# FlinkML/flink-parameter-server

Measured on NVIDIA H100. Metric: matrix-factorization updates/sec (whole box, max over ranks), higher is better.
Workload: dtype fp32

## Files before the change

### flink-parameter-server_b200/models/mf/device.py

```python
from __future__ import annotations

import math
import os
from typing import Iterable, Optional, Sequence, Tuple

import torch
import torch.distributed as dist

from ...errors import FactorIsNotANumberException
from ...ops import native
from ...utils.metrics import GLOBAL as METRICS
from ...runtime.device_stream import DevicePrefetcher
from ...store.replica_cache import ReplicaCache
from ...store.sharded_table import ShardedTable

ERR_SIGMOID = 0
ERR_PLAIN = 1

DEFAULT_DEVICE_PULL_LIMIT = 0

L2_TABLE_BYTES = 48 << 20
WINDOW_BUDGET = 256 << 20
WINDOW_BYTES_PER_ROW = 8 + 12
WINDOW_MAX_STRIDE = 128
# ... 88 lines not shown
                 flush_require: str = "any", replica_own_inplace: Optional[bool] = None,
                 output_ring=None, loss: str = "pointwise", regularization: float = 0.0,
                 step_window: Optional[int] = None, optimizer: str = "sgd",
                 negative_sampling: str = "uniform", margin: Optional[float] = None):
        self._pending = []
        self.step_window = 0
        check_negative_sampling(negative_sampling, negative_sample_rate)
        self.negative_sampling = negative_sampling
        if loss not in ("pointwise", "bpr", "warp"):
            raise ValueError(f"loss must be 'pointwise', 'bpr' or 'warp', got {loss!r}")
        self.loss, self.reg = loss, float(regularization)
        if loss == "pointwise" and self.reg != 0.0:
            raise ValueError("regularization is only supported with loss='bpr' or loss='warp'")
        self.margin = check_warp(loss, margin, optimizer=optimizer, negative_sampling=negative_sampling)
        if loss != "pointwise":
            if output_ring is not None:
                raise ValueError(f"the per-update output ring is not supported with loss={loss!r}")
            if kernel == "tma":
                raise ValueError(f"kernel='tma' is not supported with loss={loss!r}")
            if item_blocking:
                raise ValueError(f"item_blocking is not supported with loss={loss!r}")
            item_blocking = False
        self.device = torch.cuda.current_device() if device is None else int(device)
        self.cuda_device = torch.device("cuda", self.device)
        self.group = group
        ready = dist.is_available() and dist.is_initialized()
        self.world = dist.get_world_size(group) if ready else 1
        self.rank = dist.get_rank(group) if ready else 0
        if item_cache is None:
            item_cache = self.world > 1 and os.environ.get("FPS_ITEM_CACHE", "1") != "0"
        check_optimizer(optimizer, item_cache=bool(item_cache), output_ring=output_ring, kernel=kernel)
        self.optimizer = optimizer
        self.num_users, self.num_items, self.k = int(num_users), int(num_items), int(num_factors)
        self.lr = float(learning_rate)
        self.neg = int(negative_sample_rate)
        self.pull_limit = int(pull_limit)
        self.err_mode = int(err_mode)
        self.seed = int(seed)
        self.step_no = 0
        self.kernel = kernel
        self.credits = (torch.tensor([self.pull_limit, 0], dtype=torch.int32, device=self.cuda_device)
                        if self.pull_limit >= 32 and os.environ.get("FPS_STATIC_LIMITER", "0") != "1"
                        and loss == "pointwise" and optimizer == "sgd" else None)
        self.output_ring = output_ring
        with torch.cuda.device(self.device):
            self._items = ShardedTable(num_items, num_factors, partition="hash", group=group,
                                      device=self.device, init="uniform",
                                      init_range=(range_min, range_max), seed=seed * 2 + 1,
                                      track_touched=track_touched)
            n_local = -(-self.num_users // self.world)
            self._users = torch.empty((n_local, self._items.stride), dtype=torch.float32,
                                     device=self.cuda_device)
            native.init_rows(self._users, self.k, self.rank, self.world, native.PART_HASH, n_local,
                             seed * 2 + 2, range_min, range_max)
            self._stats = torch.zeros(STATS_SIZE[loss], dtype=torch.float32, device=self.cuda_device)
            self._user_acc = self._item_acc = None
            if optimizer == "adagrad":
                self._user_acc = torch.zeros(n_local, dtype=torch.float32, device=self.cuda_device)
                self._item_acc = self._items.row_accumulators()
            self._nan_flag = torch.zeros(1, dtype=torch.int32, device=self.cuda_device)
            self.user_memory = int(user_memory) if self.neg > 0 else 0
            if self.user_memory > 0:
                self.seen = torch.full((n_local, self.user_memory), -1, dtype=torch.int32,
                                       device=self.cuda_device)
                self.seen_pos = torch.zeros(n_local, dtype=torch.int32, device=self.cuda_device)
            self._registry = (native.seen_registry(self.num_items, self.cuda_device)
                              if negative_sampling == "seen" else None)
        self.item_cache = bool(item_cache)
        self.sync_every = max(1, int(sync_every))
        self.sync_interval_ms = sync_interval_ms
        self.flush_count, self.flush_require = flush_count, flush_require
        self._own_inplace = replica_own_inplace
        self.replica = (ReplicaCache(self._items, self.sync_every, sync_interval_ms,
                                     require=flush_require, flush_count=flush_count,
                                     own_inplace=replica_own_inplace)
                        if self.item_cache else None)
        row_bytes = self._items.stride * 4
        if item_blocking is None:
            item_blocking = ((self.world == 1 or self.item_cache) and self.num_items * row_bytes > (48 << 20)
                             and (self.neg == 0 or self.user_memory > 0 or negative_sampling == "seen")
                             and os.environ.get("FPS_ITEM_BLOCKING", "1") != "0")
        self.item_blocking = bool(item_blocking)
        block_bytes = int(os.environ.get("FPS_BLOCK_BYTES", block_bytes))
        self.l2_hints = self.item_blocking and os.environ.get("FPS_L2_HINTS", "0") == "1"
        per_bucket = max(1, int(block_bytes) // row_bytes)
        self.block_shift = max(0, per_bucket.bit_length() - 1)
        table_rows = self._items.rows_per_shard * self.world if self.item_cache else self.num_items
        self._table_rows = table_rows
        while -(-table_rows >> self.block_shift) > native.BUCKET_MAX:
            self.block_shift += 1
        self.block_buckets = max(1, -(-table_rows >> self.block_shift))
        if self.item_blocking:
            with torch.cuda.device(self.device):
                self._bucket_scratch = torch.zeros(2 * native.BUCKET_MAX, dtype=torch.int32,
                                                   device=self.cuda_device)
        self.step_window = step_window_size(step_window, world=self.world, item_cache=self.item_cache,
                                            loss=self.loss, table_rows=self.num_items, stride=self._items.stride,
                                            env=os.environ.get("FPS_STEP_WINDOW"), optimizer=optimizer)
        self._win = None
        self._win_phase_ns = None
        self._graph_capture = False
        self._per_launch = False
        self._items.barrier()

    @property
    def stats(self) -> torch.Tensor:
        self._drain()
        return self._stats

    @property
    def users(self) -> torch.Tensor:
        self._drain()
        return self._users

    @property
    def items(self) -> ShardedTable:
        self._drain()
        return self._items

    @property
    def nan_flag(self) -> torch.Tensor:
        self._drain()
        return self._nan_flag

    @property
    def accumulators(self) -> Optional[Tuple[torch.Tensor, torch.Tensor]]:
        self._drain()
        if self._item_acc is None:
            return None
        return self._user_acc, self._item_acc.local

    def _windowable(self, users, items, ratings) -> bool:
        if self.step_window < 2 or self._graph_capture or self._per_launch:
            return False
        packed = items is None
        return step_windowable(
            neg=self.neg, output_ring=self.output_ring, pull_limit=self.pull_limit, credits=self.credits,
            kernel=self.kernel, kernel_env=os.environ.get("FPS_MF_KERNEL", "reg"),
            reg_variant_env=os.environ.get("FPS_MF_REG_VARIANT"), l2_hints=self.l2_hints, packed=packed,
            dtypes=(users.dtype,) if packed else (users.dtype, items.dtype, ratings.dtype),
            n_records=users.numel(), table_rows=self.num_items, on_gpu=users.is_cuda,
            capturing=torch.cuda.is_current_stream_capturing())

    def _stage(self, users, items, ratings) -> None:
        if self._win is None:
            rows, w = self.num_items, self.step_window
            slot_bytes = -(-rows * 12 // 256) * 256
            with torch.cuda.device(self.device):
                dev = self.cuda_device
                self._win = {
                    "slot_bytes": slot_bytes,
                    "stage": torch.empty(w * slot_bytes, dtype=torch.uint8, device=dev),
                    "slots": torch.full((w, rows), -1, dtype=torch.int64, device=dev),
                    "user_bits": torch.zeros(-(-self._users.shape[0] // 32), dtype=torch.int32, device=dev),
                    "ctl": torch.zeros(2 * native.WINDOW_MAX, dtype=torch.int32, device=dev),
                    "slot_stats": torch.zeros((w, 2), dtype=torch.float32, device=dev),
                }
        j = len(self._pending)
        n = users.numel()
        sb = self._win["slot_bytes"]
        slot = self._win["stage"][j * sb:(j + 1) * sb]
        if items is None:
            slot[:8 * n].view(torch.int64).copy_(users.reshape(-1), non_blocking=True)
        else:
            ids = slot[:12 * n].view(torch.int32)
            ids[:n].copy_(users.reshape(-1), non_blocking=True)
            ids[n:2 * n].copy_(items.reshape(-1), non_blocking=True)
            ids[2 * n:].view(torch.float32).copy_(ratings.reshape(-1), non_blocking=True)
        self._pending.append((n, 1 if items is None else 0))
        self.step_no += 1
        METRICS.inc("mf_ratings", n)

    def _drain(self) -> int:
        n = len(self._pending)
        if n == 0:
            return 0
        counts, fmts = zip(*self._pending)
        self._pending = []
        w = self._win
        native.mf_window_drain(w["stage"], w["slot_bytes"], counts, fmts, self._users, self._items.local, self.lr,
                               self.err_mode, w["slots"], w["user_bits"], w["ctl"], self._stats, w["slot_stats"],
                               self._nan_flag, phase_ns=self._win_phase_ns)
        return n

    def flush(self) -> None:
        self._drain()
        if self.replica is not None:
            self.replica.flush()

    def step(self, users: torch.Tensor, items: Optional[torch.Tensor] = None,
             ratings: Optional[torch.Tensor] = None, negatives: Optional[torch.Tensor] = None) -> None:
        if self.loss == "pointwise" and negatives is None and self._windowable(users, items, ratings):
            self._stage(users, items, ratings)
            if len(self._pending) >= self.step_window:
                self._drain()
            return
        self._drain()
        check_negative_sampling(self.negative_sampling, self.neg, negatives)
        if self.loss != "pointwise":
            self._step_pairwise(users, items, ratings, negatives)
            return
        if negatives is not None:
            raise ValueError("negatives= needs loss='bpr' or loss='warp'")
        neg = self.neg
        if self.user_memory > 0 or self._registry is not None:
            users, items, ratings = self._sample_negatives(users, items, ratings)
            neg = 0
        n_records = users.numel()
        fed = False
        ring = self.output_ring
        out_args = ring.kernel_args() if ring is not None else None
        revisits = self.item_cache or n_records * (1 + neg) > self._table_rows
        if self.item_blocking and self.block_buckets > 1 and revisits:
            hashed = self.item_cache and self._items.mode == native.PART_HASH
            fed = hashed
            users, items, ratings = native.bucket_by_item(
                users, items, ratings, self.block_shift, self.block_buckets, self._bucket_scratch,
                num_shards=self.world if hashed else 1, rows_per_shard=self._items.rows_per_shard,
                pending=self.replica.pending if hashed else None)
        if self.item_cache:
            self.replica.after_step(n_records * (1 + neg), fed=fed)
            native.mf_sgd_fused(users, items, ratings, self._users, self.world, self.replica.table_c,
                                self.lr, err_mode=self.err_mode, neg_rate=neg,
                                num_items=self.num_items, seed=self.seed, step=self.step_no,
                                stats=self._stats, nan_flag=self._nan_flag,
                                max_inflight_rows=self.pull_limit, kernel="reg", l2_hints=self.l2_hints,
                                reserve_total=self.replica.reserve_total(), output=out_args,
                                credits=self.credits)
        else:
            native.mf_sgd_fused(users, items, ratings, self._users, self.world, self._items.table_c,
                                self.lr, err_mode=self.err_mode, neg_rate=neg,
                                num_items=self.num_items, seed=self.seed, step=self.step_no,
                                stats=self._stats, nan_flag=self._nan_flag,
                                max_inflight_rows=self.pull_limit, kernel=self.kernel,
                                l2_hints=self.l2_hints, output=out_args, credits=self.credits,
                                item_acc=self._item_acc.table_c if self._item_acc is not None else None,
                                user_acc=self._user_acc)
        if ring is not None:
            ring.after_kernel(users.numel() * (1 + neg))
        self.step_no += 1
        METRICS.inc("mf_ratings", users.numel())

    def _step_pairwise(self, users, items, ratings, negatives) -> None:
        if negatives is not None:
            if self.item_cache:
                raise ValueError("negatives= is not supported in the replica (item_cache) mode")
            n = int(negatives.shape[1]) if negatives.dim() == 2 else 0
        elif self.neg < 1:
            raise ValueError(f"loss={self.loss!r} needs negative_sample_rate >= 1 or explicit negatives=")
        elif self.user_memory > 0 or self._registry is not None:
            per = 1 + self.neg
            ou, oi, orat = self._sample_negatives(users, items, ratings)
            ou, oi = ou.view(-1, per), oi.view(-1, per)
            negatives = torch.where(ou[:, 1:] >= 0, oi[:, 1:], torch.full_like(oi[:, 1:], -1)).contiguous()
            users, items, ratings = ou[:, 0].contiguous(), oi[:, 0].contiguous(), orat.view(-1, per)[:, 0].contiguous()
            n = self.neg
        else:
            n = self.neg
        if self.output_ring is not None:
            raise ValueError(f"the per-update output ring is not supported with loss={self.loss!r}")
        n_pos = users.numel()
        cand, reserve = self._items.table_c, 0
        if self.item_cache:
            self.replica.after_step(n_pos * (n if self.loss == "bpr" else 1), fed=False)
            cand, reserve = self.replica.table_c, self.replica.reserve_total()
        if self.loss == "warp":
            native.mf_warp_fused(users, items, ratings, self._users, cand, self.lr, self.reg, margin=self.margin,
                                 rank_items=self.num_items, negatives=negatives, n_neg=n, num_items=self.num_items,
                                 seed=self.seed, step=self.step_no, anchor_div=self.world, stats=self._stats,
                                 nan_flag=self._nan_flag, max_inflight_rows=self.pull_limit, reserve_total=reserve)
            self.step_no += 1
            METRICS.inc("mf_ratings", n_pos)
            return
        native.mf_bpr_fused(users, items, ratings, self._users, cand, self.lr, self.reg, negatives=negatives,
                            n_neg=n, num_items=self.num_items, seed=self.seed, step=self.step_no,
                            anchor_div=self.world, stats=self._stats, nan_flag=self._nan_flag,
                            max_inflight_rows=self.pull_limit, reserve_total=reserve,
                            anchor_acc=self._user_acc,
                            cand_acc=self._item_acc.table_c if self._item_acc is not None else None)
        self.step_no += 1
        METRICS.inc("mf_ratings", n_pos)

    def _sample_negatives(self, users, items, ratings):
        memory = self.user_memory > 0
        if self._registry is not None:
            return native.neg_sample_seen(users, items, ratings, self.neg, self._registry,
                                          self.seen if memory else None, self.seen_pos if memory else None,
                                          self.world, seed=self.seed, step=self.step_no)
        return native.neg_sample(users, items, ratings, self.neg, self.num_items, self.seen, self.seen_pos,
                                 self.world, seed=self.seed, step=self.step_no)

    def seen_items(self) -> torch.Tensor:
        if self._registry is None:
            raise ValueError("seen_items() needs negative_sampling='seen'")
        order, count, _ = self._registry
        return order[:int(count.item())].to(torch.int64)

    def make_graph_step(self, batch_size: int, packed: bool = True):
        self._drain()
        dev = self.cuda_device
        if packed:
            static = (torch.zeros(batch_size, dtype=torch.int64, device=dev),)
        else:
            static = (torch.zeros(batch_size, dtype=torch.int32, device=dev),
                      torch.zeros(batch_size, dtype=torch.int32, device=dev),
                      torch.zeros(batch_size, dtype=torch.float32, device=dev))
        s = torch.cuda.Stream(device=dev)
        s.wait_stream(torch.cuda.current_stream(dev))
        self._graph_capture = True
        try:
            with torch.cuda.stream(s):
                for _ in range(2):
                    self._stats.zero_(); self.step(*static)
            torch.cuda.current_stream(dev).wait_stream(s)
            graph = torch.cuda.CUDAGraph()
            with torch.cuda.graph(graph, stream=s):
                self._stats.zero_()
                self.step(*static)
        finally:
            self._graph_capture = False

        def replay():
            self._drain()
            graph.replay()
        return static, replay

    def fit_stream(self, host_batches: Iterable[Sequence[torch.Tensor]],
                   loss_every: int = 1):
        self._drain()
        pf = DevicePrefetcher(host_batches, self.cuda_device, depth=2)
        self.prefetcher = pf
        pending = []
        ring = [torch.empty(self._stats.numel(), dtype=torch.float32).pin_memory() for _ in range(4)]
        i = 0
        for batch in pf:
# ... 100 lines not shown
```

### flink-parameter-server_b200/ops/csrc/fps_mf_window.cu

```cuda
#include <cuda_fp16.h>
#include <cooperative_groups.h>
#include "fps_common.cuh"
#include "fps_mf_args.cuh"

namespace cg = cooperative_groups;

#define WIN_MAX 8
#define WIN_THREADS 256
#define WIN_EMPTY 0xFFFFFFFFFFFFFFFFull

struct WinArgs {
  const unsigned char* stage;
  long long slot_bytes;
  long long n[WIN_MAX];
  int fmt[WIN_MAX];
  int n_slots;
  int err_mode;
  float lr;
  int stride;
  float* user_table;
  float* item_table;
  long long rows;
  unsigned long long* slots;
  unsigned int* user_bits;
  long long bm_words;
  unsigned int* ctl;
  float* stats;
  float* slot_stats;
  int* nan_flag;
  unsigned long long* phase_ns;
};

__device__ __forceinline__ bool win_record(const WinArgs& a, int j, long long i, int& user, int& item,
                                           float& rating) {
  const unsigned char* base = a.stage + (long long)j * a.slot_bytes;
  if (a.fmt[j] == 1) {
    const unsigned long long rec = reinterpret_cast<const unsigned long long*>(base)[i];
    user = (int)(rec >> 38);
    item = (int)((rec >> 16) & 0x3FFFFFull);
    rating = __half2float(__ushort_as_half((unsigned short)(rec & 0xFFFFull)));
    return true;
  }
  const long long n = a.n[j];
  user = reinterpret_cast<const int*>(base)[i];
  item = reinterpret_cast<const int*>(base)[n + i];
  rating = reinterpret_cast<const float*>(base)[2 * n + i];
  return user >= 0;
}

__device__ __forceinline__ float win_add(float x, float y) {
  float z;
  asm("add.rn.ftz.f32 %0, %1, %2;" : "=f"(z) : "f"(x), "f"(y));
  return z;
}
__device__ __forceinline__ float4 win_add4(float4 x, float g, float4 y) {
  return make_float4(win_add(x.x, g * y.x), win_add(x.y, g * y.y), win_add(x.z, g * y.z), win_add(x.w, g * y.w));
}

__device__ __forceinline__ unsigned long long win_clock() {
  unsigned long long t;
  asm volatile("mov.u64 %0, %%globaltimer;" : "=l"(t));
  return t;
}
__device__ __forceinline__ void win_phase(const WinArgs& a, int k) {
  const unsigned long long t = win_clock();
  a.phase_ns[k] += t - a.phase_ns[3];
  a.phase_ns[3] = t;
  if (k == 1) a.phase_ns[2] += 1ull;
}

template <int G, int NS>
__device__ __forceinline__ void win_flush_stats(const WinArgs& a, float (&sq)[NS], float (&cnt)[NS], int nr,
                                                int slot0, float* sh) {
  const int lane = threadIdx.x & (G - 1);
  __syncthreads();
  if (threadIdx.x < 2 * WIN_MAX) sh[threadIdx.x] = 0.f;
  __syncthreads();
#pragma unroll
  for (int r = 0; r < WIN_MAX; ++r) {
    if (r < nr) {
      const bool mine = lane == r % G;
      float s = mine ? sq[r / G] : 0.f, c = mine ? cnt[r / G] : 0.f;
#pragma unroll
      for (int o = 16; o > 0; o >>= 1) {
        s += __shfl_xor_sync(0xffffffffu, s, o);
        c += __shfl_xor_sync(0xffffffffu, c, o);
      }
      if ((threadIdx.x & 31) == 0 && c > 0.f) {
        atomicAdd(sh + 2 * r, s);
        atomicAdd(sh + 2 * r + 1, c);
      }
    }
  }
#pragma unroll
  for (int i = 0; i < NS; ++i) sq[i] = cnt[i] = 0.f;
  __syncthreads();
  if (threadIdx.x < 2 * nr && sh[threadIdx.x] != 0.f)
    atomicAdd(a.slot_stats + 2 * slot0 + threadIdx.x, sh[threadIdx.x]);
}

template <int G, int VPL>
__device__ __forceinline__ void win_load(float4 (&x)[VPL], const float* row, int lane, int nvec, bool on) {
#pragma unroll
  for (int k = 0; k < VPL; ++k) {
    const int c = lane + k * G;
    x[k] = (on && c < nvec) ? *reinterpret_cast<const float4*>(row + 4 * c) : make_float4(0.f, 0.f, 0.f, 0.f);
  }
}
template <int G, int VPL>
__device__ __forceinline__ void win_store(float* row, const float4 (&x)[VPL], int lane, int nvec) {
#pragma unroll
  for (int k = 0; k < VPL; ++k) {
    const int c = lane + k * G;
    if (c < nvec) *reinterpret_cast<float4*>(row + 4 * c) = x[k];
  }
}
template <int G, int VPL>
__device__ __forceinline__ float win_dot(const float4 (&u)[VPL], const float4 (&v)[VPL]) {
  float d[VPL];
#pragma unroll
  for (int k = 0; k < VPL; ++k) {
    d[k] = 0.f;
    d[k] += fps_mf_dot4(u[k], v[k]);
  }
#pragma unroll
  for (int h = VPL / 2; h > 0; h >>= 1)
#pragma unroll
    for (int k = 0; k < h; ++k) d[k] += d[k + h];
  return fps_group_sum<G>(d[0]);
}

template <int LPR, int VPL, int P, int MINB>
__global__ void __launch_bounds__(WIN_THREADS, MINB) fps_mf_window_kernel(const __grid_constant__ WinArgs a) {
  static_assert(VPL >= 1 && VPL <= LPR && LPR % VPL == 0, "VPL must divide LPR");
  constexpr int G = LPR / VPL;
  __shared__ float sh[2 * WIN_MAX];
  cg::grid_group grid = cg::this_grid();
  const int lane = threadIdx.x & (G - 1);
  const int gtid = blockIdx.x * blockDim.x + threadIdx.x;
  const int gthreads = gridDim.x * blockDim.x;
  const int group = gtid / G;
  const int n_groups = gthreads / G;
  const int stride = a.stride;
  const int nvec = stride >> 2;
  constexpr int NS = G < WIN_MAX ? WIN_MAX / G : 1;
  constexpr int NE = NS;
  float sq[NS], cnt[NS];
#pragma unroll
  for (int i = 0; i < NS; ++i) sq[i] = cnt[i] = 0.f;
  bool bad = false;
  const bool timer = a.phase_ns != nullptr && blockIdx.x == 0 && threadIdx.x == 0;

  if (blockIdx.x == 0) {
    if (threadIdx.x < 2 * WIN_MAX) a.ctl[threadIdx.x] = 0u;
    if (threadIdx.x < 2 * a.n_slots) a.slot_stats[threadIdx.x] = 0.f;
  }
  if (timer) a.phase_ns[3] = win_clock();
  int start = 0, attempt = 0;
  while (start < a.n_slots) {
    for (long long w = gtid; w < a.bm_words; w += gthreads) a.user_bits[w] = 0u;
    grid.sync();
    int end = start;
    bool clashed = false;
    while (end < a.n_slots) {
      const int j = end;
      unsigned long long* t = a.slots + (long long)(j - start) * a.rows;
      bool clash = false;
      for (long long i = gtid; i < a.n[j]; i += gthreads) {
        int user, item;
        float rating;
        if (!win_record(a, j, i, user, item, rating)) continue;
        const unsigned long long e = ((unsigned long long)__float_as_uint(rating) << 32) | (unsigned int)user;
        clash |= atomicExch(t + item, e) != WIN_EMPTY;
        const unsigned int bit = 1u << (user & 31);
        clash |= (atomicOr(a.user_bits + (user >> 5), bit) & bit) != 0u;
      }
      if (clash) *reinterpret_cast<volatile unsigned int*>(a.ctl + attempt) = 1u;
      grid.sync();
      clashed = *reinterpret_cast<volatile unsigned int*>(a.ctl + attempt) != 0u;
      ++attempt;
      if (clashed) break;
      ++end;
    }
    if (timer) win_phase(a, 0);
    const int nrow = end - start;
    const int written = nrow + (clashed ? 1 : 0);
    if (nrow > 0) {
      unsigned long long nxt[NE];
#pragma unroll
      for (int m = 0; m < NE; ++m) {
        const int r = lane + m * G;
        nxt[m] = (group < a.rows && r < written) ? a.slots[(long long)r * a.rows + group] : WIN_EMPTY;
      }
      for (long long base = 0; base < a.rows; base += n_groups) {
        const long long item = base + group;
        const bool in = item < a.rows;
        float* vp = a.item_table + (in ? item : 0) * (long long)stride;
        float4 v[VPL];
#pragma unroll
        for (int k = 0; k < VPL; ++k) v[k] = make_float4(0.f, 0.f, 0.f, 0.f);
        bool any = false;
        bool loaded = false;
        unsigned long long mine[NE];
#pragma unroll
        for (int m = 0; m < NE; ++m) {
          const int r = lane + m * G;
          mine[m] = nxt[m];
          const long long it2 = item + n_groups;
          nxt[m] = (it2 < a.rows && r < written) ? a.slots[(long long)r * a.rows + it2] : WIN_EMPTY;
          if (mine[m] != WIN_EMPTY) a.slots[(long long)r * a.rows + item] = WIN_EMPTY;
        }
        const int src0 = (threadIdx.x & 31) & ~(G - 1);
#pragma unroll
        for (int c0 = 0; c0 < WIN_MAX; c0 += P) {
          if (c0 < nrow) {
            unsigned long long ent[P];
#pragma unroll
            for (int q = 0; q < P; ++q) {
              const int r = c0 + q;
              ent[q] = __shfl_sync(0xffffffffu, mine[(r / G) % NE], src0 + r % G);
              if (r >= nrow) ent[q] = WIN_EMPTY;
            }
            {
              bool chunk_any = false;
#pragma unroll
              for (int q = 0; q < P; ++q) chunk_any |= ent[q] != WIN_EMPTY;
              if (chunk_any && !loaded) win_load<G, VPL>(v, vp, lane, nvec, true);
              loaded |= chunk_any;
              any |= chunk_any;
              float4 u[P][VPL];
#pragma unroll
              for (int q = 0; q < P; ++q)
                win_load<G, VPL>(u[q], a.user_table + (long long)(unsigned int)ent[q] * stride, lane, nvec,
                                 ent[q] != WIN_EMPTY);
#pragma unroll
              for (int q = 0; q < P; ++q) {
                const int r = c0 + q;
                if (r < nrow) {
                  const float d = win_dot<G, VPL>(u[q], v);
                  const bool ok = ent[q] != WIN_EMPTY;
                  const float rating = __uint_as_float((unsigned int)(ent[q] >> 32));
                  const float resid = rating - d;
                  const float g = fps_mf_grad(a.err_mode, a.lr, rating, d, resid);
                  if (ok) {
                    if (!(fabsf(g) <= 3.0e38f)) bad = true;
                    if (lane == r % G) {
                      sq[r / G] += resid * resid;
                      cnt[r / G] += 1.f;
                    }
                    float4 nu[VPL];
#pragma unroll
                    for (int k = 0; k < VPL; ++k) {
                      nu[k] = win_add4(u[q][k], g, v[k]);
                      v[k] = win_add4(v[k], g, u[q][k]);
                    }
                    win_store<G, VPL>(a.user_table + (long long)(unsigned int)ent[q] * stride, nu, lane, nvec);
                  }
                }
              }
            }
          }
        }
        if (any) win_store<G, VPL>(vp, v, lane, nvec);
      }
      win_flush_stats<G, NS>(a, sq, cnt, nrow, start, sh);
    } else {
      const int j = start;
      unsigned long long* t = a.slots;
      for (long long base = 0; base < a.n[j]; base += n_groups) {
        const long long i = base + group;
        int user = 0, item = 0;
        float rating = 0.f;
        const bool ok = i < a.n[j] && win_record(a, j, i, user, item, rating);
        float* up = a.user_table + (long long)user * stride;
        float* vp = a.item_table + (long long)item * stride;
        float4 u[VPL], v[VPL];
#pragma unroll
        for (int k = 0; k < VPL; ++k) {
          const int c = lane + k * G;
          u[k] = v[k] = make_float4(0.f, 0.f, 0.f, 0.f);
          if (ok && c < nvec) {
            v[k] = fps_ld_row4(vp + 4 * c);
            u[k] = *reinterpret_cast<const float4*>(up + 4 * c);
          }
        }
        const float d = win_dot<G, VPL>(u, v);
        const float resid = rating - d;
        const float g = fps_mf_grad(a.err_mode, a.lr, rating, d, resid);
        if (ok) {
          if (!(fabsf(g) <= 3.0e38f)) bad = true;
          if (lane == 0) {
            sq[0] += resid * resid;
            cnt[0] += 1.f;
            t[item] = WIN_EMPTY;
          }
#pragma unroll
          for (int k = 0; k < VPL; ++k) {
            const int c = lane + k * G;
            if (c < nvec) {
              fps_red_add4(up + 4 * c, make_float4(g * v[k].x, g * v[k].y, g * v[k].z, g * v[k].w));
              fps_red_add4(vp + 4 * c, make_float4(g * u[k].x, g * u[k].y, g * u[k].z, g * u[k].w));
            }
          }
        }
      }
      win_flush_stats<G, NS>(a, sq, cnt, 1, start, sh);
      end = start + 1;
    }
    grid.sync();
    if (timer) win_phase(a, 1);
    start = end;
  }
  if (bad && a.nan_flag != nullptr) *a.nan_flag = 1;
  if (blockIdx.x == 0 && threadIdx.x == 0 && a.stats != nullptr) {
    float s = 0.f, c = 0.f;
    for (int j = 0; j < a.n_slots; ++j) {
      s += a.slot_stats[2 * j];
      c += a.slot_stats[2 * j + 1];
    }
    a.stats[0] += s;
    a.stats[1] += c;
  }
}

template <int LPR, int VPL, int P, int MINB>
static int launch_window(const WinArgs& a, int num_sms, cudaStream_t stream) {
  constexpr int V = VPL < LPR ? VPL : LPR;
  int occ = 0;
  cudaError_t e =
      cudaOccupancyMaxActiveBlocksPerMultiprocessor(&occ, fps_mf_window_kernel<LPR, V, P, MINB>, WIN_THREADS, 0);
  if (e != cudaSuccess) return (int)e;
  if (occ < 1) return -1402;
  const long long grid = (long long)num_sms * occ;
  WinArgs args = a;
  void* params[] = {&args};
  e = cudaLaunchCooperativeKernel((const void*)fps_mf_window_kernel<LPR, V, P, MINB>, dim3((unsigned)grid),
                                  dim3(WIN_THREADS), params, 0, stream);
  if (e != cudaSuccess) return (int)e;
  return (int)cudaGetLastError();
}

static int g_win_variant = 0;
extern "C" void fps_set_mf_window_variant(int v) { g_win_variant = v; }

template <int LPR>
static int dispatch_window(const WinArgs& a, int num_sms, cudaStream_t s) {
  constexpr int MINB_V1 = LPR <= 2 ? 2 : 3;
  switch (g_win_variant) {
    case 1: return launch_window<LPR, 1, 8, 1>(a, num_sms, s);
    case 2: return launch_window<LPR, 1, 4, MINB_V1>(a, num_sms, s);
    default:
      if constexpr (LPR == 16) return launch_window<16, 4, 2, 2>(a, num_sms, s);
      else return launch_window<LPR, 1, 4, MINB_V1>(a, num_sms, s);
  }
}

extern "C" int fps_mf_window_drain(const WinArgs* a, int num_sms, cudaStream_t stream) {
  if (a->n_slots <= 0) return 0;
  if (a->n_slots > WIN_MAX) return -1401;
  const int nvec = a->stride >> 2;
  if (nvec <= 1) return dispatch_window<1>(*a, num_sms, stream);
  if (nvec <= 2) return dispatch_window<2>(*a, num_sms, stream);
  if (nvec <= 4) return dispatch_window<4>(*a, num_sms, stream);
  if (nvec <= 8) return dispatch_window<8>(*a, num_sms, stream);
  if (nvec <= 16) return dispatch_window<16>(*a, num_sms, stream);
  if (nvec <= 32) return dispatch_window<32>(*a, num_sms, stream);
  return -1400;
}
```

### flink-parameter-server_b200/ops/native.py

```python
from __future__ import annotations

import ctypes as C
import math
import os
import threading
from typing import Optional

import torch

from . import build as _build

FPS_MAX_SHARDS = 16
PART_HASH = 0
PART_RANGE = 1
PART_LUT = 2
LUT_OWNER_SHIFT = 40

_lib = None
_lib_lock = threading.Lock()
_launch_count = 0


class ShardTableC(C.Structure):

# ... 161 lines not shown

class _RawCudaBuffer:

    def __init__(self, ptr: int, shape, typestr: str):
        self.__cuda_array_interface__ = {
            "shape": tuple(shape),
            "typestr": typestr,
            "data": (int(ptr), False),
            "version": 3,
            "strides": None,
        }


_TYPESTR = {torch.float32: "<f4", torch.int32: "<i4", torch.int64: "<i8", torch.uint8: "|u1",
            torch.float16: "<f2", torch.int16: "<i2"}


def tensor_from_ptr(ptr: int, shape, dtype: torch.dtype, device: int) -> torch.Tensor:
    if dtype == torch.bfloat16:
        t = torch.as_tensor(_RawCudaBuffer(ptr, shape, "<i2"), device=torch.device("cuda", device))
        return t.view(torch.bfloat16)
    return torch.as_tensor(_RawCudaBuffer(ptr, shape, _TYPESTR[dtype]),
                           device=torch.device("cuda", device))


def init_rows(rows: torch.Tensor, dim: int, shard: int, num_shards: int, mode: int, div: int,
              seed: int, lo: float, hi: float) -> None:
    _req(rows, "rows", torch.float32)
    n_rows, stride = rows.shape
    assert stride % 4 == 0
    _check(lib().fps_init_rows(C.c_void_p(rows.data_ptr()), C.c_longlong(n_rows), int(dim),
                               int(stride), int(shard), int(num_shards), int(mode),
                               C.c_longlong(div), C.c_ulonglong(seed & (2**64 - 1)),
                               C.c_float(lo), C.c_float(hi), _stream()), "init_rows")
    _bump()


MF_ERR_MODES = (0, 1, 2)


def _check_pointwise(users, items, ratings, err_mode) -> None:
    if int(err_mode) not in MF_ERR_MODES:
        raise ValueError(f"err_mode must be one of {MF_ERR_MODES}, got {err_mode!r}")
    if items is None:
        if users.dtype != torch.int64:
            raise TypeError("packed rating records must be an int64 tensor (see pack_ratings)")
        return
    if users.dtype != items.dtype:
        raise TypeError("users and items must share an integer dtype")
    if items.numel() != users.numel() or ratings.numel() != users.numel():
        raise ValueError("users, items and ratings must have the same length")


def mf_sgd_fused(users: torch.Tensor, items: torch.Tensor, ratings: torch.Tensor,
                 user_table, user_div: int, item_tab: ShardTableC, lr: float,
                 err_mode: int = 0, neg_rate: int = 0, num_items: int = 0, seed: int = 0,
                 step: int = 0, stats: Optional[torch.Tensor] = None,
                 nan_flag: Optional[torch.Tensor] = None, max_inflight_rows: int = 0,
                 kernel: Optional[str] = None, push_tab: Optional[ShardTableC] = None,
                 l2_hints: bool = False, reserve_ctas: int = 0, reserve_total: int = 0,
                 progress: Optional[torch.Tensor] = None, output=None,
                 credits: Optional[torch.Tensor] = None, item_acc: Optional[ShardTableC] = None,
                 user_acc=None) -> None:
    _check_pointwise(users, items, ratings, err_mode)
    if int(neg_rate) > 0 and int(num_items) < 2:
        raise ValueError(f"sampled negatives need num_items >= 2, got {num_items}")
    _req(users, "users")
    user_sharded = isinstance(user_table, ShardTableC)
    if not user_sharded:
        _req(user_table, "user_table", torch.float32)
    packed = items is None
    if not packed:
        _req(items, "items"); _req(ratings, "ratings", torch.float32)
    if (user_table.stride if user_sharded else user_table.shape[1]) != item_tab.stride:
        raise ValueError("user table stride must equal item table stride")
    a = MfArgsC()
    a.users = users.data_ptr()
    a.items = None if packed else items.data_ptr()
    a.ratings = None if packed else ratings.data_ptr()
    a.format = 1 if packed else 0
    a.n_pos = users.numel(); a.neg_rate = int(neg_rate); a.num_items = int(max(num_items, 1))
    a.seed = seed & (2**64 - 1); a.step = int(step)
    if user_sharded:
        a.user_table = None; a.user_tab = user_table; a.user_sharded = 1
    else:
        a.user_table = user_table.data_ptr(); a.user_sharded = 0
    a.user_div = int(user_div)
    a.user_shift = log2_or_neg(int(user_div))
    a.lr = float(lr); a.err_mode = int(err_mode)
    a.stats = stats.data_ptr() if stats is not None else None
    a.nan_flag = nan_flag.data_ptr() if nan_flag is not None else None
    a.item_tab = item_tab
    if push_tab is not None:
        a.push_tab = push_tab; a.use_push_tab = 1
    a.l2_hints = 1 if l2_hints else 0
    variant = kernel or os.environ.get("FPS_MF_KERNEL", "reg")
    if packed or push_tab is not None or l2_hints or output is not None or credits is not None:
        variant = "reg"
    a.progress = progress.data_ptr() if progress is not None else None
    if credits is not None:
        _req(credits, "credits", torch.int32)
        a.credits = credits.data_ptr()
    if output is not None:
        o_ids, o_vecs, o_staged, o_cap, o_every = output
        a.out_ids = o_ids.data_ptr(); a.out_vecs = o_vecs.data_ptr(); a.out_staged = o_staged.data_ptr()
        a.out_cap = int(o_cap); a.out_every = int(o_every)
    if item_acc is not None:
        if push_tab is not None or output is not None or credits is not None:
            raise ValueError("row-wise AdaGrad does not support push_tab, output or credits")
        if int(item_acc.stride) != 1:
            raise ValueError("item_acc must be a stride-1 accumulator table")
        a.item_acc = item_acc
        if user_sharded:
            if not isinstance(user_acc, ShardTableC) or int(user_acc.stride) != 1:
                raise ValueError("a sharded user table needs a stride-1 ShardTableC user_acc")
            a.user_acc_tab = user_acc
        else:
            if not torch.is_tensor(user_acc):
                raise ValueError("a worker-local user table needs a float32 user_acc tensor")
            _req(user_acc, "user_acc", torch.float32)
            if user_acc.numel() < user_table.shape[0]:
                raise ValueError("user_acc must hold one accumulator per user row")
            a.user_acc = user_acc.data_ptr()
        variant = "reg"
    elif user_acc is not None:
        raise ValueError("user_acc needs item_acc")
    lib().fps_set_mf_reserve(int(reserve_ctas))
    lib().fps_set_mf_reserve_total(int(reserve_total))
    rv = os.environ.get("FPS_MF_REG_VARIANT")
    if rv is not None:
        lib().fps_set_mf_reg_variant(int(rv))
    if variant == "tma":
        code = lib().fps_mf_sgd_tma(C.byref(a), _id_bytes(users), int(max_inflight_rows),
                                    sm_count(users.device.index), _stream())
        if code != -1002:
            _check(code, "mf_sgd_tma")
            _bump()
            return
    _check(lib().fps_mf_sgd_fused(C.byref(a), 4 if packed else _id_bytes(users), int(max_inflight_rows),
                                  sm_count(users.device.index), _stream()), "mf_sgd_fused")
    _bump()


WINDOW_MAX = 8


class WinArgsC(C.Structure):

    _fields_ = [
        ("stage", C.c_void_p), ("slot_bytes", C.c_longlong),
        ("n", C.c_longlong * WINDOW_MAX), ("fmt", C.c_int * WINDOW_MAX),
        ("n_slots", C.c_int), ("err_mode", C.c_int), ("lr", C.c_float), ("stride", C.c_int),
        ("user_table", C.c_void_p), ("item_table", C.c_void_p), ("rows", C.c_longlong),
        ("slots", C.c_void_p), ("user_bits", C.c_void_p), ("bm_words", C.c_longlong),
        ("ctl", C.c_void_p), ("stats", C.c_void_p), ("slot_stats", C.c_void_p), ("nan_flag", C.c_void_p),
        ("phase_ns", C.c_void_p),
    ]


def mf_window_drain(stage: torch.Tensor, slot_bytes: int, counts, formats, user_table: torch.Tensor,
                    item_table: torch.Tensor, lr: float, err_mode: int, slots: torch.Tensor,
                    user_bits: torch.Tensor, ctl: torch.Tensor, stats: torch.Tensor, slot_stats: torch.Tensor,
                    nan_flag: torch.Tensor, phase_ns: Optional[torch.Tensor] = None) -> None:
    n = len(counts)
    if not 0 < n <= WINDOW_MAX or len(formats) != n:
        raise ValueError(f"1..{WINDOW_MAX} staged micro-batches expected, got {n}")
    for t, name in ((stage, "stage"), (user_table, "user_table"), (item_table, "item_table"), (slots, "slots"),
                    (user_bits, "user_bits"), (ctl, "ctl"), (stats, "stats"), (slot_stats, "slot_stats"),
                    (nan_flag, "nan_flag")):
        _req(t, name)
    if user_table.shape[1] != item_table.shape[1]:
        raise ValueError("user table stride must equal item table stride")
    if user_bits.numel() * 32 < user_table.shape[0] or slots.numel() < n * item_table.shape[0]:
        raise ValueError("user bitmap or slot table too small")
    if slot_stats.numel() < 2 * n or ctl.numel() < 2 * WINDOW_MAX:
        raise ValueError("slot_stats / ctl too small")
    a = WinArgsC()
    a.stage = stage.data_ptr(); a.slot_bytes = int(slot_bytes)
    for j in range(n):
        a.n[j] = int(counts[j]); a.fmt[j] = int(formats[j])
    a.n_slots = n; a.err_mode = int(err_mode); a.lr = float(lr); a.stride = int(item_table.shape[1])
    a.user_table = user_table.data_ptr(); a.item_table = item_table.data_ptr(); a.rows = int(item_table.shape[0])
    a.slots = slots.data_ptr(); a.user_bits = user_bits.data_ptr(); a.bm_words = user_bits.numel()
    a.ctl = ctl.data_ptr(); a.stats = stats.data_ptr(); a.slot_stats = slot_stats.data_ptr()
    a.nan_flag = nan_flag.data_ptr()
    if phase_ns is not None:
        _req(phase_ns, "phase_ns", torch.int64)
        if phase_ns.numel() < 4:
            raise ValueError("phase_ns too small")
        a.phase_ns = phase_ns.data_ptr()
    rv = os.environ.get("FPS_MF_WINDOW_VARIANT")
    if rv is not None:
        lib().fps_set_mf_window_variant(int(rv))
    _check(lib().fps_mf_window_drain(C.byref(a), sm_count(stage.device.index), _stream()), "mf_window_drain")
    _bump()


class BprArgsC(C.Structure):

    _fields_ = [
        ("users", C.c_void_p), ("items", C.c_void_p), ("ratings", C.c_void_p), ("negatives", C.c_void_p),
        ("n_pos", C.c_longlong), ("n_neg", C.c_int), ("format", C.c_int),
        ("num_items", C.c_longlong), ("seed", C.c_ulonglong), ("step", C.c_ulonglong),
        ("lr", C.c_float), ("reg", C.c_float),
        ("anchor_table", C.c_void_p), ("anchor_div", C.c_int), ("anchor_shift", C.c_int),
        ("anchor_sharded", C.c_int), ("cand_sharded", C.c_int), ("anchor_tab", ShardTableC),
        ("cand_table", C.c_void_p), ("cand_div", C.c_int), ("cand_shift", C.c_int), ("cand_tab", ShardTableC),
        ("use_push_tab", C.c_int), ("stride", C.c_int), ("push_tab", ShardTableC),
        ("stats", C.c_void_p), ("nan_flag", C.c_void_p), ("reserve_total", C.c_int), ("pad_", C.c_int),
        ("anchor_acc_tab", ShardTableC), ("cand_acc", ShardTableC), ("anchor_acc", C.c_void_p),
        ("rank_items", C.c_longlong), ("margin", C.c_float), ("pad2_", C.c_int),
    ]


def _pairwise_args(users, items, ratings, anchor_table, cand_table, lr, reg, negatives, n_neg, num_items, seed,
                   step, anchor_div, cand_div, stats, n_stats, nan_flag, push_tab, reserve_total):
    _req(users, "users")
    packed = items is None
    if packed:
        if users.dtype != torch.int64:
            raise TypeError("packed rating records must be an int64 tensor (see pack_ratings)")
        id_dtype = torch.int32
    else:
        _req(items, "items"); _req(ratings, "ratings", torch.float32)
        if users.dtype != items.dtype:
            raise TypeError("users and items must share an integer dtype")
        if items.numel() != users.numel() or ratings.numel() != users.numel():
            raise ValueError("users, items and ratings must have the same length")
        id_dtype = users.dtype
    n_pos = users.numel()
    a = BprArgsC()
    strides = []
    for name, tab, div in (("anchor", anchor_table, anchor_div), ("cand", cand_table, cand_div)):
        if isinstance(tab, ShardTableC):
            setattr(a, f"{name}_tab", tab); setattr(a, f"{name}_sharded", 1)
            strides.append(int(tab.stride))
        else:
            _req(tab, f"{name}_table", torch.float32)
            setattr(a, f"{name}_table", tab.data_ptr())
            setattr(a, f"{name}_div", int(div)); setattr(a, f"{name}_shift", log2_or_neg(int(div)))
            strides.append(int(tab.shape[1]))
    if strides[0] != strides[1]:
        raise ValueError("anchor table stride must equal candidate table stride")
    a.stride = strides[0]
    if push_tab is not None:
        if not a.cand_sharded:
            raise ValueError("push_tab needs a ShardTable cand_table")
        if int(push_tab.stride) != a.stride:
            raise ValueError("push table stride must equal candidate table stride")
        a.push_tab = push_tab; a.use_push_tab = 1
    if negatives is not None:
        _req(negatives, "negatives", id_dtype)
        if negatives.dim() != 2 or negatives.shape[0] != n_pos:
            raise ValueError(f"negatives must be [{n_pos}, n]")
        a.negatives = negatives.data_ptr(); a.n_neg = int(negatives.shape[1])
    else:
        if int(n_neg) < 1:
            raise ValueError("n_neg must be >= 1 when negatives are sampled")
        if int(num_items) < 2:
            raise ValueError(f"sampled negatives need num_items >= 2, got {num_items}")
        a.n_neg = int(n_neg)
    if stats is not None:
        _req(stats, "stats", torch.float32)
        if stats.numel() < n_stats:
            raise ValueError(f"stats must hold {n_stats} floats")
        a.stats = stats.data_ptr()
    if nan_flag is not None:
        _req(nan_flag, "nan_flag", torch.int32)
        a.nan_flag = nan_flag.data_ptr()
    a.users = users.data_ptr()
    a.items = None if packed else items.data_ptr()
    a.ratings = None if packed else ratings.data_ptr()
    a.format = 1 if packed else 0
    a.n_pos = n_pos; a.num_items = int(max(num_items, 1))
    a.seed = seed & (2**64 - 1); a.step = int(step)
    a.lr = float(lr); a.reg = float(reg); a.reserve_total = int(reserve_total)
    return a, packed


def mf_bpr_fused(users: torch.Tensor, items: Optional[torch.Tensor], ratings: Optional[torch.Tensor],
                 anchor_table, cand_table, lr: float, reg: float = 0.0, *,
                 negatives: Optional[torch.Tensor] = None, n_neg: int = 1, num_items: int = 0,
                 seed: int = 0, step: int = 0, anchor_div: int = 1, cand_div: int = 1,
                 stats: Optional[torch.Tensor] = None, nan_flag: Optional[torch.Tensor] = None,
                 max_inflight_rows: int = 0, push_tab: Optional[ShardTableC] = None,
                 reserve_total: int = 0, anchor_acc=None, cand_acc: Optional[ShardTableC] = None) -> None:
    a, packed = _pairwise_args(users, items, ratings, anchor_table, cand_table, lr, reg, negatives, n_neg, num_items,
                               seed, step, anchor_div, cand_div, stats, 3, nan_flag, push_tab, reserve_total)
    if cand_acc is not None:
        if not a.cand_sharded or push_tab is not None:
            raise ValueError("row-wise AdaGrad needs a ShardTableC cand_table and no push_tab")
        if int(cand_acc.stride) != 1:
            raise ValueError("cand_acc must be a stride-1 accumulator table")
        a.cand_acc = cand_acc
        if a.anchor_sharded:
            if not isinstance(anchor_acc, ShardTableC) or int(anchor_acc.stride) != 1:
                raise ValueError("a sharded anchor table needs a stride-1 ShardTableC anchor_acc")
            a.anchor_acc_tab = anchor_acc
        else:
            if not torch.is_tensor(anchor_acc):
                raise ValueError("a worker-local anchor table needs a float32 anchor_acc tensor")
            _req(anchor_acc, "anchor_acc", torch.float32)
            if anchor_acc.numel() < anchor_table.shape[0]:
                raise ValueError("anchor_acc must hold one accumulator per anchor row")
            a.anchor_acc = anchor_acc.data_ptr()
    elif anchor_acc is not None:
        raise ValueError("anchor_acc needs cand_acc")
    _check(lib().fps_mf_bpr_fused(C.byref(a), 4 if packed else _id_bytes(users), int(max_inflight_rows),
                                  sm_count(users.device.index), _stream()), "mf_bpr_fused")
    _bump()


WARP_TRIAL_BLOCKS = (1, 2, 4, 8)


def mf_warp_fused(users: torch.Tensor, items: Optional[torch.Tensor], ratings: Optional[torch.Tensor],
                  anchor_table, cand_table, lr: float, reg: float = 0.0, *, margin: float = 1.0,
                  rank_items: int = 0, negatives: Optional[torch.Tensor] = None, n_neg: int = 1,
                  num_items: int = 0, seed: int = 0, step: int = 0, anchor_div: int = 1, cand_div: int = 1,
                  stats: Optional[torch.Tensor] = None, nan_flag: Optional[torch.Tensor] = None,
                  max_inflight_rows: int = 0, push_tab: Optional[ShardTableC] = None, reserve_total: int = 0,
                  trial_block: int = 0) -> None:
    if not math.isfinite(float(margin)):
        raise ValueError(f"margin must be finite, got {margin!r}")
    if int(trial_block) not in (0,) + WARP_TRIAL_BLOCKS:
        raise ValueError(f"trial_block must be 0 or one of {WARP_TRIAL_BLOCKS}, got {trial_block!r}")
    a, packed = _pairwise_args(users, items, ratings, anchor_table, cand_table, lr, reg, negatives, n_neg, num_items,
                               seed, step, anchor_div, cand_div, stats, 4, nan_flag, push_tab, reserve_total)
    a.margin = float(margin)
    a.rank_items = int(rank_items) if int(rank_items) > 0 else int(a.num_items)
    _check(lib().fps_mf_warp_fused(C.byref(a), 4 if packed else _id_bytes(users), int(trial_block),
                                   int(max_inflight_rows), sm_count(users.device.index), _stream()), "mf_warp_fused")
    _bump()


def init_rows_f64(rows: torch.Tensor, dim: int, shard: int, num_shards: int, mode: int, div: int, seed: int,
                  lo: float, hi: float) -> None:
    _req(rows, "rows", torch.float64)
    _check(lib().fps_init_rows_f64(C.c_void_p(rows.data_ptr()), C.c_longlong(rows.shape[0]), int(dim),
                                   int(rows.shape[1]), int(shard), int(num_shards), int(mode), C.c_longlong(div),
                                   C.c_ulonglong(seed & (2**64 - 1)), C.c_double(lo), C.c_double(hi), _stream()),
           "init_rows_f64")
    _bump()
# ... 758 lines not shown
```

Measured before the change: 3.297 billion.

## Detect window clashes in one grid pass using per-user slot bytes and epoch tags

Conflict detection changes from one grid.sync per staged micro-batch to a single scatter pass over all slots. Each user gets a byte mask of the slots that touched it, and item slot entries carry an epoch tag bit, so the earliest clashing slot is found with an atomicMax. Stale entries from the previous drain are told apart by the tag and cleared lazily, and the user mask is zeroed with vectorised stores after each round instead of a separate pass. This cuts grid-wide barriers and atomics, but it scatters every slot even when an early slot clashes, and it adds extra timing probes and cross-call epoch and prev_rows state.

Measured after the change: 3.298 billion (median of 6 runs). No clear change (+0.0%).

```diff
diff --git a/flink-parameter-server_b200/models/mf/device.py b/flink-parameter-server_b200/models/mf/device.py
--- a/flink-parameter-server_b200/models/mf/device.py
+++ b/flink-parameter-server_b200/models/mf/device.py
@@ -264,9 +264,10 @@
                     "slot_bytes": slot_bytes,
                     "stage": torch.empty(w * slot_bytes, dtype=torch.uint8, device=dev),
                     "slots": torch.full((w, rows), -1, dtype=torch.int64, device=dev),
-                    "user_bits": torch.zeros(-(-self._users.shape[0] // 32), dtype=torch.int32, device=dev),
+                    "user_mask": torch.zeros(-(-self._users.shape[0] // 16) * 16, dtype=torch.uint8, device=dev),
                     "ctl": torch.zeros(2 * native.WINDOW_MAX, dtype=torch.int32, device=dev),
                     "slot_stats": torch.zeros((w, 2), dtype=torch.float32, device=dev),
+                    "epoch": 0, "prev_rows": 0,
                 }
         j = len(self._pending)
         n = users.numel()
@@ -291,8 +292,10 @@
         self._pending = []
         w = self._win
         native.mf_window_drain(w["stage"], w["slot_bytes"], counts, fmts, self._users, self._items.local, self.lr,
-                               self.err_mode, w["slots"], w["user_bits"], w["ctl"], self._stats, w["slot_stats"],
-                               self._nan_flag, phase_ns=self._win_phase_ns)
+                               self.err_mode, w["slots"], w["user_mask"], w["ctl"], self._stats, w["slot_stats"],
+                               self._nan_flag, phase_ns=self._win_phase_ns, epoch=w["epoch"],
+                               prev_rows=w["prev_rows"])
+        w["epoch"], w["prev_rows"] = 1 - w["epoch"], n
         return n
 
     def flush(self) -> None:
diff --git a/flink-parameter-server_b200/ops/csrc/fps_mf_window.cu b/flink-parameter-server_b200/ops/csrc/fps_mf_window.cu
--- a/flink-parameter-server_b200/ops/csrc/fps_mf_window.cu
+++ b/flink-parameter-server_b200/ops/csrc/fps_mf_window.cu
@@ -8,6 +8,7 @@
 #define WIN_MAX 8
 #define WIN_THREADS 256
 #define WIN_EMPTY 0xFFFFFFFFFFFFFFFFull
+#define WIN_TAG (1ull << 31)
 
 struct WinArgs {
   const unsigned char* stage;
@@ -22,13 +23,16 @@
   float* item_table;
   long long rows;
   unsigned long long* slots;
-  unsigned int* user_bits;
-  long long bm_words;
+  unsigned char* user_mask;
+  long long user_mask_bytes;
   unsigned int* ctl;
   float* stats;
   float* slot_stats;
   int* nan_flag;
   unsigned long long* phase_ns;
+  int phase_len;
+  int epoch;
+  int prev_rows;
 };
 
 __device__ __forceinline__ bool win_record(const WinArgs& a, int j, long long i, int& user, int& item,
@@ -67,6 +71,13 @@
   a.phase_ns[k] += t - a.phase_ns[3];
   a.phase_ns[3] = t;
   if (k == 1) a.phase_ns[2] += 1ull;
+  if (a.phase_len >= 8) a.phase_ns[7] = t;
+}
+__device__ __forceinline__ void win_detail(const WinArgs& a, int k) {
+  if (a.phase_len < 8) return;
+  const unsigned long long t = win_clock();
+  if (k >= 0) a.phase_ns[k] += t - a.phase_ns[7];
+  a.phase_ns[7] = t;
 }
 
 template <int G, int NS>
@@ -151,40 +162,39 @@
   bool bad = false;
   const bool timer = a.phase_ns != nullptr && blockIdx.x == 0 && threadIdx.x == 0;
 
-  if (blockIdx.x == 0) {
-    if (threadIdx.x < 2 * WIN_MAX) a.ctl[threadIdx.x] = 0u;
-    if (threadIdx.x < 2 * a.n_slots) a.slot_stats[threadIdx.x] = 0.f;
-  }
-  if (timer) a.phase_ns[3] = win_clock();
-  int start = 0, attempt = 0;
+  if (blockIdx.x == 0 && threadIdx.x < 2 * a.n_slots) a.slot_stats[threadIdx.x] = 0.f;
+  if (timer) {
+    a.phase_ns[3] = win_clock();
+    if (a.phase_len >= 8) a.phase_ns[7] = a.phase_ns[3];
+  }
+  int start = 0;
   while (start < a.n_slots) {
-    for (long long w = gtid; w < a.bm_words; w += gthreads) a.user_bits[w] = 0u;
-    grid.sync();
-    int end = start;
-    bool clashed = false;
-    while (end < a.n_slots) {
-      const int j = end;
+    unsigned int* user_words = reinterpret_cast<unsigned int*>(a.user_mask);
+    int cand = WIN_MAX;
+    const unsigned long long tag = a.epoch ? WIN_TAG : 0ull;
+    for (int j = start; j < a.n_slots; ++j) {
       unsigned long long* t = a.slots + (long long)(j - start) * a.rows;
-      bool clash = false;
       for (long long i = gtid; i < a.n[j]; i += gthreads) {
         int user, item;
         float rating;
         if (!win_record(a, j, i, user, item, rating)) continue;
-        const unsigned long long e = ((unsigned long long)__float_as_uint(rating) << 32) | (unsigned int)user;
-        clash |= atomicExch(t + item, e) != WIN_EMPTY;
-        const unsigned int bit = 1u << (user & 31);
-        clash |= (atomicOr(a.user_bits + (user >> 5), bit) & bit) != 0u;
-      }
-      if (clash) *reinterpret_cast<volatile unsigned int*>(a.ctl + attempt) = 1u;
-      grid.sync();
-      clashed = *reinterpret_cast<volatile unsigned int*>(a.ctl + attempt) != 0u;
-      ++attempt;
-      if (clashed) break;
-      ++end;
-    }
+        const unsigned long long e = ((unsigned long long)__float_as_uint(rating) << 32) | (unsigned int)user | tag;
+        const unsigned long long old = atomicExch(t + item, e);
+        if (old != WIN_EMPTY && (old & WIN_TAG) == tag) cand = min(cand, j);
+        const int sh_u = 8 * (user & 3);
+        const unsigned int ub = (atomicOr(user_words + (user >> 2), 1u << (sh_u + j)) >> sh_u) & 0xFFu;
+        if (ub != 0u) cand = min(cand, max(j, __ffs(ub) - 1));
+      }
+    }
+    if (cand < WIN_MAX) atomicMax(a.ctl + start, (unsigned int)(WIN_MAX - cand));
+    if (timer) win_detail(a, 5);
+    grid.sync();
+    if (timer) win_detail(a, 6);
+    const unsigned int first_clash = *reinterpret_cast<volatile unsigned int*>(a.ctl + start);
+    int end = first_clash != 0u ? WIN_MAX - (int)first_clash : a.n_slots;
     if (timer) win_phase(a, 0);
     const int nrow = end - start;
-    const int written = nrow + (clashed ? 1 : 0);
+    const int written = max(a.n_slots - start, a.prev_rows);
     if (nrow > 0) {
       unsigned long long nxt[NE];
 #pragma unroll
@@ -208,7 +218,9 @@
           mine[m] = nxt[m];
           const long long it2 = item + n_groups;
           nxt[m] = (it2 < a.rows && r < written) ? a.slots[(long long)r * a.rows + it2] : WIN_EMPTY;
-          if (mine[m] != WIN_EMPTY) a.slots[(long long)r * a.rows + item] = WIN_EMPTY;
+          const bool cur = mine[m] != WIN_EMPTY && ((mine[m] & WIN_TAG) != 0ull) == (a.epoch != 0);
+          if (mine[m] != WIN_EMPTY && (!cur || end < a.n_slots)) a.slots[(long long)r * a.rows + item] = WIN_EMPTY;
+          mine[m] = cur ? (mine[m] & ~WIN_TAG) : WIN_EMPTY;
         }
         const int src0 = (threadIdx.x & 31) & ~(G - 1);
 #pragma unroll
@@ -266,7 +278,6 @@
       win_flush_stats<G, NS>(a, sq, cnt, nrow, start, sh);
     } else {
       const int j = start;
-      unsigned long long* t = a.slots;
       for (long long base = 0; base < a.n[j]; base += n_groups) {
         const long long i = base + group;
         int user = 0, item = 0;
@@ -292,7 +303,6 @@
           if (lane == 0) {
             sq[0] += resid * resid;
             cnt[0] += 1.f;
-            t[item] = WIN_EMPTY;
           }
 #pragma unroll
           for (int k = 0; k < VPL; ++k) {
@@ -305,12 +315,20 @@
         }
       }
       win_flush_stats<G, NS>(a, sq, cnt, 1, start, sh);
+      for (long long w = gtid; w < (long long)written * a.rows; w += gthreads) a.slots[w] = WIN_EMPTY;
       end = start + 1;
     }
+    if (timer) win_detail(a, -1);
+    {
+      uint4* q = reinterpret_cast<uint4*>(a.user_mask);
+      for (long long w = gtid; w < (a.user_mask_bytes >> 4); w += gthreads) q[w] = make_uint4(0u, 0u, 0u, 0u);
+    }
+    if (timer) win_detail(a, 4);
     grid.sync();
     if (timer) win_phase(a, 1);
     start = end;
   }
+  if (blockIdx.x == 0 && threadIdx.x < a.n_slots) a.ctl[threadIdx.x] = 0u;
   if (bad && a.nan_flag != nullptr) *a.nan_flag = 1;
   if (blockIdx.x == 0 && threadIdx.x == 0 && a.stats != nullptr) {
     float s = 0.f, c = 0.f;
diff --git a/flink-parameter-server_b200/ops/native.py b/flink-parameter-server_b200/ops/native.py
--- a/flink-parameter-server_b200/ops/native.py
+++ b/flink-parameter-server_b200/ops/native.py
@@ -337,27 +337,31 @@
         ("n", C.c_longlong * WINDOW_MAX), ("fmt", C.c_int * WINDOW_MAX),
         ("n_slots", C.c_int), ("err_mode", C.c_int), ("lr", C.c_float), ("stride", C.c_int),
         ("user_table", C.c_void_p), ("item_table", C.c_void_p), ("rows", C.c_longlong),
-        ("slots", C.c_void_p), ("user_bits", C.c_void_p), ("bm_words", C.c_longlong),
+        ("slots", C.c_void_p), ("user_mask", C.c_void_p), ("user_mask_bytes", C.c_longlong),
         ("ctl", C.c_void_p), ("stats", C.c_void_p), ("slot_stats", C.c_void_p), ("nan_flag", C.c_void_p),
-        ("phase_ns", C.c_void_p),
+        ("phase_ns", C.c_void_p), ("phase_len", C.c_int), ("epoch", C.c_int), ("prev_rows", C.c_int),
     ]
 
 
 def mf_window_drain(stage: torch.Tensor, slot_bytes: int, counts, formats, user_table: torch.Tensor,
                     item_table: torch.Tensor, lr: float, err_mode: int, slots: torch.Tensor,
-                    user_bits: torch.Tensor, ctl: torch.Tensor, stats: torch.Tensor, slot_stats: torch.Tensor,
-                    nan_flag: torch.Tensor, phase_ns: Optional[torch.Tensor] = None) -> None:
+                    user_mask: torch.Tensor, ctl: torch.Tensor, stats: torch.Tensor, slot_stats: torch.Tensor,
+                    nan_flag: torch.Tensor, phase_ns: Optional[torch.Tensor] = None, *, epoch: int,
+                    prev_rows: int) -> None:
     n = len(counts)
     if not 0 < n <= WINDOW_MAX or len(formats) != n:
         raise ValueError(f"1..{WINDOW_MAX} staged micro-batches expected, got {n}")
     for t, name in ((stage, "stage"), (user_table, "user_table"), (item_table, "item_table"), (slots, "slots"),
-                    (user_bits, "user_bits"), (ctl, "ctl"), (stats, "stats"), (slot_stats, "slot_stats"),
+                    (ctl, "ctl"), (stats, "stats"), (slot_stats, "slot_stats"),
                     (nan_flag, "nan_flag")):
         _req(t, name)
     if user_table.shape[1] != item_table.shape[1]:
         raise ValueError("user table stride must equal item table stride")
-    if user_bits.numel() * 32 < user_table.shape[0] or slots.numel() < n * item_table.shape[0]:
-        raise ValueError("user bitmap or slot table too small")
+    _req(user_mask, "user_mask", torch.uint8)
+    if user_mask.numel() < user_table.shape[0] or slots.numel() < n * item_table.shape[0]:
+        raise ValueError("user mask or slot table too small")
+    if user_mask.numel() % 16 or user_mask.data_ptr() % 16:
+        raise ValueError("user_mask must be 16-byte aligned with a size that is a multiple of 16")
     if slot_stats.numel() < 2 * n or ctl.numel() < 2 * WINDOW_MAX:
         raise ValueError("slot_stats / ctl too small")
     a = WinArgsC()
@@ -366,14 +370,17 @@
         a.n[j] = int(counts[j]); a.fmt[j] = int(formats[j])
     a.n_slots = n; a.err_mode = int(err_mode); a.lr = float(lr); a.stride = int(item_table.shape[1])
     a.user_table = user_table.data_ptr(); a.item_table = item_table.data_ptr(); a.rows = int(item_table.shape[0])
-    a.slots = slots.data_ptr(); a.user_bits = user_bits.data_ptr(); a.bm_words = user_bits.numel()
+    a.slots = slots.data_ptr(); a.user_mask = user_mask.data_ptr(); a.user_mask_bytes = user_mask.numel()
     a.ctl = ctl.data_ptr(); a.stats = stats.data_ptr(); a.slot_stats = slot_stats.data_ptr()
+    if epoch not in (0, 1) or not 0 <= prev_rows <= slots.numel() // max(1, item_table.shape[0]):
+        raise ValueError("epoch must be 0 or 1 and prev_rows within the slot table")
+    a.epoch = int(epoch); a.prev_rows = int(prev_rows)
     a.nan_flag = nan_flag.data_ptr()
     if phase_ns is not None:
         _req(phase_ns, "phase_ns", torch.int64)
         if phase_ns.numel() < 4:
             raise ValueError("phase_ns too small")
-        a.phase_ns = phase_ns.data_ptr()
+        a.phase_ns = phase_ns.data_ptr(); a.phase_len = phase_ns.numel()
     rv = os.environ.get("FPS_MF_WINDOW_VARIANT")
     if rv is not None:
         lib().fps_set_mf_window_variant(int(rv))
```
